# somepago/DCR

Hardware: NVIDIA H100
Metric: embed+top-k query images/sec (higher is better)
Workload: dtype bf16

## Files before the change

dcr_b200/csrc/conv3x3_halo.cu:

```cuda
#include <cuda_bf16.h>

#include <algorithm>
#include <cstring>

#include "dcr_internal.cuh"
#include "host_util.cuh"
#include "ptx.cuh"

namespace dcr {

namespace {

constexpr int kHM = 128;
constexpr int kHK = 64;
constexpr int kSlabBytes = kHM * 128;
constexpr int kHThreads = 288;

struct HaloMaps {
  CUtensorMap a;
  CUtensorMap w;
  CUtensorMap out;
};

struct HaloParams {
  int H, W, Wp, R, N, cblocks;
  int tiles_per_img, num_tiles;
  int a_bufs, w_stages;
  uint32_t halo_bytes;
  uint32_t a_buf_bytes;
  const float* scale;
  const float* bias;
// ... 2 lines not shown

DCR_DEVICE void tma_store_commit_() { asm volatile("cp.async.bulk.commit_group;" ::: "memory"); }
DCR_DEVICE void tma_store_wait_read_() { asm volatile("cp.async.bulk.wait_group.read 0;" ::: "memory"); }
DCR_DEVICE void tma_store_wait_all_() { asm volatile("cp.async.bulk.wait_group 0;" ::: "memory"); }
DCR_DEVICE uint32_t pack_bf16_(float a, float b) {
  __nv_bfloat162 p = __floats2bfloat162_rn(a, b);
  return *reinterpret_cast<uint32_t*>(&p);
}

template <int BN, bool kRW>
__global__ void __launch_bounds__(kHThreads, 1)
    conv3x3_halo_kernel(const __grid_constant__ HaloMaps maps, const HaloParams p) {
  extern __shared__ __align__(1024) uint8_t smem_raw[];
  uint8_t* smem = reinterpret_cast<uint8_t*>((reinterpret_cast<uintptr_t>(smem_raw) + 1023) & ~uintptr_t(1023));
  constexpr int kWStage = BN * 128;
  constexpr int kChunksPerWarp = BN / 64;
  uint8_t* a_ring = smem;
  uint8_t* w_ring = a_ring + p.a_bufs * p.a_buf_bytes;
  uint8_t* out_stage = w_ring + (kRW ? 9 * p.cblocks : p.w_stages) * kWStage;
  uint8_t* acc_xpose = out_stage + (BN / 64) * kSlabBytes;
  float* sb = reinterpret_cast<float*>(acc_xpose + 8 * kAccXposeWarpBytes);
  uint64_t* bars = reinterpret_cast<uint64_t*>(sb + 2 * BN);
  uint64_t* a_full = bars;
  uint64_t* a_empty = bars + 4;
  uint64_t* w_full = bars + 8;
  uint64_t* w_empty = bars + 16;

  const uint32_t warp = threadIdx.x >> 5, lane = threadIdx.x & 31;
  if (warp == 8 && lane == 0) {
    tma_prefetch_desc(&maps.a);
    tma_prefetch_desc(&maps.w);
    tma_prefetch_desc(&maps.out);
  }
  if (warp == 0 && lane == 0) {
    for (int s = 0; s < p.a_bufs; ++s) {
      mbar_init(&a_full[s], 1);
      mbar_init(&a_empty[s], 8);
    }
    for (int s = 0; s < (kRW ? 1 : p.w_stages); ++s) {
      mbar_init(&w_full[s], 1);
      mbar_init(&w_empty[s], 8);
    }
    fence_mbar_init();
  }
  __syncthreads();

  if (warp == 8) {
    {
      PipeState as(p.a_bufs), ws(kRW ? 1 : p.w_stages);
      if constexpr (kRW) {
        if (elect_one()) {
          mbar_arrive_expect_tx(&w_full[0], 9 * p.cblocks * kWStage);
          for (int t = 0; t < 9 * p.cblocks; ++t)
            tma_load_2d(w_ring + t * kWStage, &maps.w, &w_full[0], t * kHK, 0, kEvictLast);
        }
        __syncwarp();
      }
      for (int tile = blockIdx.x; tile < p.num_tiles; tile += gridDim.x) {
        const int b = tile / p.tiles_per_img;
        const int p0 = (tile - b * p.tiles_per_img) * p.R;
        for (int cb = 0; cb < p.cblocks; ++cb, as.next()) {
          const uint32_t sa = as.s, pha = as.ph;
          mbar_wait(&a_empty[sa], pha ^ 1);
// ... 4 lines not shown
          __syncwarp();
          if constexpr (kRW) continue;
          for (int tap = 0; tap < 9; ++tap, ws.next()) {
            const uint32_t sw = ws.s, phw = ws.ph;
            mbar_wait(&w_empty[sw], phw ^ 1);
            if (elect_one()) {
              mbar_arrive_expect_tx(&w_full[sw], kWStage);
              tma_load_2d(w_ring + sw * kWStage, &maps.w, &w_full[sw], (tap * p.cblocks + cb) * kHK, 0, kEvictLast);
            }
            __syncwarp();
          }
        }
      }
    }
  } else {
    const uint32_t ewarp = warp;
    const uint32_t quad = warp & 3;
    const uint32_t half = ewarp >> 2;
    const uint32_t m = quad * 32 + lane;
    const uint32_t etid = ewarp * 32 + lane;
    const uint32_t xacc = smem_u32(acc_xpose) + warp * kAccXposeWarpBytes;
    const uint32_t a_base = smem_u32(a_ring);
    const uint32_t w_base = smem_u32(w_ring) + half * (BN / 2) * 128;
    const uint32_t row_bytes = static_cast<uint32_t>(p.Wp) * 128u;
    PipeState as(p.a_bufs), ws(kRW ? 1 : p.w_stages);
    if constexpr (kRW) mbar_wait(&w_full[0], 0);
    const int pl = static_cast<int>(m) / p.Wp, ql = static_cast<int>(m) - pl * p.Wp;
    const bool valid = ql < p.W && pl < p.R;
    const uint32_t srow = static_cast<uint32_t>(pl * p.W + ql);
    const uint32_t sb_addr = smem_u32(sb), stage_addr = smem_u32(out_stage);
    for (int c = etid; c < BN; c += 256) {
      st_shared_f32(sb_addr + c * 4, (p.scale && c < p.N) ? p.scale[c] : 1.f);
      st_shared_f32(sb_addr + (BN + c) * 4, (p.bias && c < p.N) ? p.bias[c] : 0.f);
    }
    for (int tile = blockIdx.x; tile < p.num_tiles; tile += gridDim.x) {
      const int b = tile / p.tiles_per_img;
      const int p0 = (tile - b * p.tiles_per_img) * p.R;
      if (etid == 0) tma_store_wait_read_();
      asm volatile("bar.sync 1, 256;" ::: "memory");
      WgAcc<BN / 2> acc;
      uint32_t accumulate = 0;
      for (int cb = 0; cb < p.cblocks; ++cb, as.next()) {
        const uint32_t sa = as.s;
        mbar_wait(&a_full[sa], as.ph);
        const uint32_t a_buf = a_base + sa * p.a_buf_bytes;
#pragma unroll 1
        for (int tap = 0; tap < 9; ++tap) {
          const int r = tap / 3, s = tap - 3 * r;
          uint32_t sw = 0;
          if constexpr (!kRW) {
            sw = ws.s;
            mbar_wait(&w_full[sw], ws.ph);
          } else {
            sw = static_cast<uint32_t>(tap * p.cblocks + cb);
          }
          const uint32_t a_addr = a_buf + r * row_bytes + s * 128u;
          const uint32_t b_addr = w_base + sw * kWStage;
          wgmma_fence();
#pragma unroll
          for (int k = 0; k < kHK / 16; ++k) acc.mma(a_addr + 32 * k, wgmma_desc_sw128(b_addr + 32 * k), accumulate | k);
          wgmma_commit();
          wgmma_wait<0>();
          accumulate = 1;
          if constexpr (!kRW) {
            if (lane == 0) mbar_arrive(&w_empty[sw]);
            ws.next();
          }
        }
        if (lane == 0) mbar_arrive(&a_empty[sa]);
      }
      acc.fence_regs();
#pragma unroll
      for (int ci = 0; ci < kChunksPerWarp; ++ci) {
        const int ch = half * kChunksPerWarp + ci;
        uint32_t r[32];
        acc.rows32(ci, r, xacc, lane);
        if (ch * 32 >= p.N) continue;
        float y[32];
#pragma unroll
        for (int c = 0; c < 32; c += 4) {
          const float4 sc = ld_shared_f4(sb_addr + (ch * 32 + c) * 4);
          const float4 bi = ld_shared_f4(sb_addr + (BN + ch * 32 + c) * 4);
          y[c + 0] = fmaf(__uint_as_float(r[c + 0]), sc.x, bi.x);
          y[c + 1] = fmaf(__uint_as_float(r[c + 1]), sc.y, bi.y);
          y[c + 2] = fmaf(__uint_as_float(r[c + 2]), sc.z, bi.z);
          y[c + 3] = fmaf(__uint_as_float(r[c + 3]), sc.w, bi.w);
        }
        if (p.act == 1) {
#pragma unroll
          for (int c = 0; c < 32; ++c) y[c] = fmaxf(y[c], 0.f);
        }
        const uint32_t dst = stage_addr + (ch >> 1) * kSlabBytes + srow * 128;
        const uint32_t sw = srow & 7;
#pragma unroll
        for (int j = 0; j < 4; ++j) {
          uint4 v;
          v.x = pack_bf16_(y[j * 8 + 0], y[j * 8 + 1]);
          v.y = pack_bf16_(y[j * 8 + 2], y[j * 8 + 3]);
          v.z = pack_bf16_(y[j * 8 + 4], y[j * 8 + 5]);
          v.w = pack_bf16_(y[j * 8 + 6], y[j * 8 + 7]);
          if (valid) st_shared_v4(dst + ((((ch & 1) * 4 + j) ^ sw) << 4), v);
        }
        __syncwarp();
      }
      fence_proxy_async();
      asm volatile("bar.sync 2, 256;" ::: "memory");
      if (etid == 0) {
        for (int sl = 0; sl < BN / 64; ++sl)
          if (sl * 64 < p.N) tma_store_4d(&maps.out, out_stage + sl * kSlabBytes, p.out_col_off + sl * 64, 0, p0, b);
        tma_store_commit_();
      }
    }
    if (etid == 0) tma_store_wait_all_();
  }

}

template <int BN, bool kRW>
int launch_halo(const HaloMaps& maps, HaloParams& p, int num_sms, size_t max_smem, cudaStream_t stream) {
  constexpr size_t kWStage = static_cast<size_t>(BN) * 128;
  const size_t fixed = 1024 + static_cast<size_t>(BN / 64) * kSlabBytes + 8 * kAccXposeWarpBytes + 2 * BN * 4 + 256;
  const size_t abuf = p.a_buf_bytes;
  size_t smem = 0;
  if constexpr (kRW) {
    const size_t wres = static_cast<size_t>(9) * p.cblocks * kWStage;
    DCR_REQUIRE(max_smem >= fixed + wres + 2 * abuf, "conv3x3_halo: resident weights do not fit");
    p.a_bufs = static_cast<int>(std::min<size_t>(4, (max_smem - fixed - wres) / abuf));
    p.w_stages = 0;
    smem = fixed + wres + static_cast<size_t>(p.a_bufs) * abuf;
  } else {
    p.a_bufs = 2;
    DCR_REQUIRE(max_smem >= fixed + 2 * abuf + 3 * kWStage, "conv3x3_halo: not enough shared memory");
    p.w_stages = static_cast<int>(std::min<size_t>(8, (max_smem - fixed - 2 * abuf) / kWStage));
    if (max_smem >= fixed + 3 * abuf + 6 * kWStage) {
      p.a_bufs = 3;
      p.w_stages = static_cast<int>(std::min<size_t>(8, (max_smem - fixed - 3 * abuf) / kWStage));
// ... 59 lines not shown
```

dcr_b200/csrc/conv_gemm.cu:

```cuda
#include <cuda_bf16.h>

#include <algorithm>
#include <cstring>

#include "dcr_internal.cuh"
#include "host_util.cuh"
#include "ptx.cuh"

namespace dcr {

namespace {

constexpr int kBM = 128;
constexpr int kBK = 64;
constexpr int kThreads = 288;
constexpr int kAccXposeBytes = 8 * kAccXposeWarpBytes;
constexpr int kAStage = kBM * kBK * 2;
constexpr int kXposePitch = 80;
constexpr int kXposeWarpBytes = 32 * kXposePitch;
constexpr int kXposeBytes = 8 * kXposeWarpBytes;

struct GemmMaps {
  CUtensorMap a[3];
  CUtensorMap w[3];
  CUtensorMap out;
  CUtensorMap res;
};

struct GemmParams {
  int M, N;
// ... 2 lines not shown
  int term_a[kMaxGemmTerms], term_w[kMaxGemmTerms];
  int P, Q, stride, pad_h, pad_w;
  int num_m_tiles, num_n_tiles, stages;
  const float* scale;
  const float* bias;
  const __nv_bfloat16* res;
  int ld_res, res_planes;
  long long res_plane_stride;
  __nv_bfloat16* out;
  int ld_out, out_col_off, out_planes;
  long long out_plane_stride;
  float* out_f32;
  int ld_out_f32;
  int act;
  int tma_epi;
  int n_out_bufs;
  int n_res_bufs;
  int fast_gelu;
  int n_fastest;
  int a_resident;
};

DCR_DEVICE float gelu_erf_fast(float y) {
  const float ax = fabsf(y) * 0.70710678118654752440f;
  float t;
  asm("rcp.approx.ftz.f32 %0, %1;" : "=f"(t) : "f"(fmaf(0.3275911f, ax, 1.f)));
  float e;
  asm("ex2.approx.ftz.f32 %0, %1;" : "=f"(e) : "f"(-1.4426950408889634f * ax * ax));
  float poly = fmaf(1.061405429f, t, -1.453152027f);
  poly = fmaf(poly, t, 1.421413741f);
  poly = fmaf(poly, t, -0.284496736f);
  poly = fmaf(poly, t, 0.254829592f);
// ... 29 lines not shown
               : "memory");
}
DCR_DEVICE void tma_store_commit() { asm volatile("cp.async.bulk.commit_group;" ::: "memory"); }
DCR_DEVICE void tma_store_wait_read() { asm volatile("cp.async.bulk.wait_group.read 0;" ::: "memory"); }
DCR_DEVICE void tma_store_wait_all() { asm volatile("cp.async.bulk.wait_group 0;" ::: "memory"); }

template <int BN, bool kIm2col, int kEpi>
__global__ void __launch_bounds__(kThreads, 1)
    gemm_bf16_kernel(const __grid_constant__ GemmMaps maps, const GemmParams p) {
  extern __shared__ __align__(1024) uint8_t smem_raw[];
  uint8_t* smem = reinterpret_cast<uint8_t*>((reinterpret_cast<uintptr_t>(smem_raw) + 1023) & ~uintptr_t(1023));
  constexpr bool kTma = kEpi != 0;
  constexpr int kBStage = BN * kBK * 2;
  constexpr int kStageBytes = kAStage + kBStage;
  constexpr int kStagingBytes = (BN / 64) * kBM * 128;
  constexpr int kChunksPerWarp = BN / 64;
  const int stages = p.stages;
  const int k_iters = p.n_terms * p.taps * p.cblocks;
  const bool a_res = p.a_resident != 0;
  const int stage_bytes = a_res ? kBStage : kStageBytes;
  const int num_n_tiles = p.num_n_tiles;
  uint8_t* smem_ares = smem;
  uint8_t* smem_ab = smem + (a_res ? k_iters * kAStage : 0);
  uint8_t* out_stage = smem_ab + stages * stage_bytes;
  uint8_t* res_stage = out_stage + (kTma ? p.n_out_bufs * kStagingBytes : kXposeBytes);
  uint8_t* acc_xpose = res_stage + p.n_res_bufs * kStagingBytes;
  float* sb = reinterpret_cast<float*>(acc_xpose + kAccXposeBytes);
  uint64_t* bars = reinterpret_cast<uint64_t*>(sb + (a_res ? 2 * num_n_tiles * BN : 4 * BN));
  uint64_t* full = bars;
  uint64_t* empty = bars + 12;
  uint64_t* res_full = bars + 28;
  uint64_t* a_full = bars + 10;
  uint64_t* a_empty = bars + 11;

  const uint32_t warp = threadIdx.x >> 5, lane = threadIdx.x & 31;
  const int M = p.M, N = p.N, num_m_tiles = p.num_m_tiles;
  const bool has_res = p.res != nullptr;
  const int num_tiles = num_m_tiles * p.num_n_tiles;
  const int unit = static_cast<int>(blockIdx.x), n_units = static_cast<int>(gridDim.x);
  const int t_first = a_res ? static_cast<int>(static_cast<long long>(num_tiles) * blockIdx.x / gridDim.x) : unit;
  const int t_end = a_res ? static_cast<int>(static_cast<long long>(num_tiles) * (blockIdx.x + 1) / gridDim.x) : num_tiles;
  const int t_step = a_res ? 1 : n_units;
  const bool n_fast = p.n_fastest != 0;
  auto tile_m = [&](int t) {
    return a_res ? t / num_n_tiles : (n_fast ? t / num_n_tiles : t % num_m_tiles);
  };
  auto tile_n = [&](int t) { return (a_res || n_fast) ? t % num_n_tiles : t / num_m_tiles; };

  if (warp == 8 && lane == 0) {
    tma_prefetch_desc(&maps.out);
    tma_prefetch_desc(&maps.res);
    for (int i = 0; i < 3; ++i) {
      tma_prefetch_desc(&maps.a[i]);
      tma_prefetch_desc(&maps.w[i]);
    }
  }
  if (warp == 0 && lane == 0) {
    for (int s = 0; s < stages; ++s) {
      mbar_init(&full[s], 1);
      mbar_init(&empty[s], 8);
    }
    for (int b = 0; b < 2; ++b) mbar_init(&res_full[b], 1);
    mbar_init(a_full, 1);
    mbar_init(a_empty, 8);
    fence_mbar_init();
  }
  __syncthreads();

  if (warp == 8) {
    {
      const int n_terms = p.n_terms, taps = p.taps, kw = p.kw, cblocks = p.cblocks;
      PipeState st(stages);
      int res_m = -1;
      uint32_t a_seg = 0;
      for (int tile = t_first; tile < t_end; tile += t_step) {
        const int m0 = tile_m(tile) * kBM;
        const int n0 = tile_n(tile) * BN;
        if (a_res) {
          if (m0 != res_m) {
            res_m = m0;
            mbar_wait(a_empty, (a_seg & 1) ^ 1);
            if (elect_one()) {
              mbar_arrive_expect_tx(a_full, k_iters * kAStage);
              for (int ki = 0; ki < k_iters; ++ki)
                tma_load_2d(smem_ares + ki * kAStage, &maps.a[p.term_a[0]], a_full, ki * kBK, m0, kEvictFirst);
            }
            __syncwarp();
            ++a_seg;
          }
          for (int ki = 0; ki < k_iters; ++ki, st.next()) {
            const uint32_t s = st.s;
            mbar_wait(&empty[s], st.ph ^ 1);
            if (elect_one()) {
              mbar_arrive_expect_tx(&full[s], kBStage);
              tma_load_2d(smem_ab + s * kBStage, &maps.w[p.term_w[0]], &full[s], ki * kBK, n0, kEvictLast);
            }
            __syncwarp();
          }
          continue;
        }
// ... 19 lines not shown
                uint8_t* sa = smem_ab + s * kStageBytes;
                if constexpr (kIm2col) {
                  tma_load_im2col_4d(sa, ma, &full[s], cb * kBK, w0, h0, img, static_cast<uint16_t>(sx),
                                          static_cast<uint16_t>(r));
                } else
                  tma_load_2d(sa, ma, &full[s], cb * kBK, m0, kEvictNormal);
                tma_load_2d(sa + kAStage, mw, &full[s], (tap * cblocks + cb) * kBK, n0, kEvictNormal);
              }
              __syncwarp();
            }
          }
        }
      }
    }
  } else {
    const uint32_t ewarp = warp;
    const uint32_t quad = warp & 3;
    const uint32_t half = ewarp >> 2;
    const uint32_t row = quad * 32 + lane;
    const uint32_t etid = ewarp * 32 + lane;
    const uint32_t xacc = smem_u32(acc_xpose) + warp * kAccXposeWarpBytes;
    const int act = p.act;
    uint32_t tc = 0;
    PipeState st(stages);
    const uint32_t a_base = smem_u32(a_res ? smem_ares : smem_ab);
    const uint32_t b_base = smem_u32(a_res ? smem_ab : smem_ab + kAStage) + half * (BN / 2) * 128;
    int res_m_c = -1;
    uint32_t a_seg = 0;
    auto load_residual = [&](int tile_idx, uint32_t rbuf) {
      const int rm0 = tile_m(tile_idx) * kBM;
      const int rn0 = tile_n(tile_idx) * BN;
      int slabs = 0;
      for (int sl = 0; sl < BN / 64; ++sl)
        if (rn0 + sl * 64 < N) ++slabs;
      mbar_arrive_expect_tx(&res_full[rbuf], slabs * kBM * 128);
      for (int sl = 0; sl < BN / 64; ++sl)
        if (rn0 + sl * 64 < N)
          tma_load_2d(res_stage + rbuf * kStagingBytes + sl * kBM * 128, &maps.res, &res_full[rbuf], rn0 + sl * 64, rm0,
                         kEvictFirst);
    };
    if (kTma && has_res && etid == 0 && t_first < t_end) load_residual(t_first, 0);
    const bool two_out = p.n_out_bufs == 2;
    const uint32_t sb_addr = smem_u32(sb), out_addr = smem_u32(out_stage), res_addr = smem_u32(res_stage);
    int staged_n0 = -1;
    uint32_t sbsel = 1;
    if (a_res) {
      const int npad = num_n_tiles * BN;
      for (int c = etid; c < npad; c += 256) {
        st_shared_f32(sb_addr + c * 4, (p.scale && c < N) ? p.scale[c] : 1.f);
        st_shared_f32(sb_addr + (npad + c) * 4, (p.bias && c < N) ? p.bias[c] : 0.f);
      }
      asm volatile("bar.sync 1, 256;" ::: "memory");
    }
    for (int tile = t_first; tile < t_end; tile += t_step, ++tc) {
      const int m0 = tile_m(tile) * kBM;
      const int n0 = tile_n(tile) * BN;
      uint8_t* ostage = out_stage + (two_out ? (tc & 1) : 0) * kStagingBytes;
      const uint32_t ostage_addr = out_addr + (two_out ? (tc & 1) : 0) * kStagingBytes;
      const uint32_t rstage_addr = res_addr + (tc & 1) * kStagingBytes;
      if constexpr (kTma) {
        if (etid == 0) {
          if (!two_out) tma_store_wait_read();
          if (has_res && tile + t_step < t_end) load_residual(tile + t_step, (tc & 1) ^ 1);
        }
      }
      const bool restage = !a_res && n0 != staged_n0;
      if (restage) {
        sbsel ^= 1;
        staged_n0 = n0;
        for (int c = etid; c < BN; c += 256) {
          const int n = n0 + c;
          st_shared_f32(sb_addr + (sbsel * 2 * BN + c) * 4, (p.scale && n < N) ? p.scale[n] : 1.f);
          st_shared_f32(sb_addr + (sbsel * 2 * BN + BN + c) * 4, (p.bias && n < N) ? p.bias[n] : 0.f);
        }
      }
      if (restage || (kTma && !two_out)) asm volatile("bar.sync 1, 256;" ::: "memory");
      const uint32_t s_scale = a_res ? sb_addr + n0 * 4 : sb_addr + sbsel * 2 * BN * 4;
      const uint32_t s_bias = s_scale + (a_res ? num_n_tiles * BN : BN) * 4;
      bool last_of_m = false;
      if (a_res) {
        const int mt = tile_m(tile);
        if (mt != res_m_c) {
          res_m_c = mt;
          mbar_wait(a_full, a_seg & 1);
          ++a_seg;
        }
        last_of_m = (tile + t_step >= t_end) || tile_m(tile + t_step) != mt;
      }
      WgAcc<BN / 2> acc;
      uint32_t prev_s = 0;
      for (int ki = 0; ki < k_iters; ++ki, st.next()) {
        const uint32_t s = st.s;
        mbar_wait(&full[s], st.ph);
        const uint32_t a_addr = a_base + (a_res ? static_cast<uint32_t>(ki) * kAStage : s * kStageBytes);
        const uint32_t b_addr = b_base + s * static_cast<uint32_t>(stage_bytes);
        wgmma_fence();
#pragma unroll
        for (int k = 0; k < kBK / 16; ++k) acc.mma(a_addr + 32 * k, wgmma_desc_sw128(b_addr + 32 * k), (ki | k) != 0);
        wgmma_commit();
        wgmma_wait<1>();
        if (ki > 0 && lane == 0) mbar_arrive(&empty[prev_s]);
        prev_s = s;
      }
      wgmma_wait<0>();
      acc.fence_regs();
      if (lane == 0) {
        mbar_arrive(&empty[prev_s]);
        if (last_of_m) mbar_arrive(a_empty);
      }
      if (kTma && has_res) mbar_wait(&res_full[tc & 1], (tc >> 1) & 1);
      const int m = m0 + static_cast<int>(row);
      const bool row_ok = m < M;
#pragma unroll
      for (int ci = 0; ci < kChunksPerWarp; ++ci) {
        const int ch = half * kChunksPerWarp + ci;
        uint32_t r[32];
        acc.rows32(ci, r, xacc, lane);
        const int nc = n0 + ch * 32;
        if (nc >= N) continue;
        float y[32];
#pragma unroll
        for (int c = 0; c < 32; c += 4) {
          const float4 sc = ld_shared_f4(s_scale + (ch * 32 + c) * 4);
          const float4 bi = ld_shared_f4(s_bias + (ch * 32 + c) * 4);
          y[c + 0] = fmaf(__uint_as_float(r[c + 0]), sc.x, bi.x);
          y[c + 1] = fmaf(__uint_as_float(r[c + 1]), sc.y, bi.y);
          y[c + 2] = fmaf(__uint_as_float(r[c + 2]), sc.z, bi.z);
          y[c + 3] = fmaf(__uint_as_float(r[c + 3]), sc.w, bi.w);
        }
        if constexpr (kTma) {
          const uint32_t srow = ostage_addr + (ch >> 1) * kBM * 128 + row * 128;
          const uint32_t rrow = rstage_addr + (ch >> 1) * kBM * 128 + row * 128;
          const uint32_t sw = row & 7;
          if (has_res) {
#pragma unroll
            for (int j = 0; j < 4; ++j) {
              const uint4 rv = ld_shared_v4(rrow + ((((ch & 1) * 4 + j) ^ sw) << 4));
              const uint32_t w[4] = {rv.x, rv.y, rv.z, rv.w};
#pragma unroll
              for (int e = 0; e < 4; ++e) {
                y[j * 8 + 2 * e] += __uint_as_float(w[e] << 16);
                y[j * 8 + 2 * e + 1] += __uint_as_float(w[e] & 0xffff0000u);
              }
            }
          }
#pragma unroll
          for (int c = 0; c < 32; ++c) y[c] = (kEpi == 3) ? gelu_tanh_fast(y[c]) : apply_act(y[c], kEpi - 1);
#pragma unroll
          for (int j = 0; j < 4; ++j) {
            uint4 v;
            v.x = pack_bf16(y[j * 8 + 0], y[j * 8 + 1]);
            v.y = pack_bf16(y[j * 8 + 2], y[j * 8 + 3]);
// ... 72 lines not shown
                const int piece = t * 32 + static_cast<int>(lane), r = piece >> 2, part = piece & 3;
                if (m_w0 + r < M && part * 8 < nvalid)
                  *reinterpret_cast<uint4*>(obase + static_cast<size_t>(m_w0 + r) * p.ld_out + part * 8) =
                      ld_shared_v4(xw + r * kXposePitch + part * 16);
              }
              if (pl + 1 < p.out_planes) {
#pragma unroll
                for (int c = 0; c < 32; ++c) y[c] -= __bfloat162float(__float2bfloat16_rn(y[c]));
              }
            }
          }
        }
      }
      if constexpr (kTma) {
        fence_proxy_async();
        if (two_out && etid == 0) tma_store_wait_read();
        asm volatile("bar.sync 2, 256;" ::: "memory");
        if (etid == 0) {
          for (int sl = 0; sl < BN / 64; ++sl)
            if (n0 + sl * 64 < N && m0 < M) tma_store_2d(&maps.out, ostage + sl * kBM * 128, p.out_col_off + n0 + sl * 64, m0);
          tma_store_commit();
        }
      }
    }
  }

  if (kTma && warp == 0 && lane == 0) tma_store_wait_all();
}

bool wants_a_resident(const GemmParams& p, int BN, bool im2col, size_t max_smem) {
  const int k_iters_h = p.n_terms * p.taps * p.cblocks;
  if (!(!im2col && p.tma_epi && p.n_terms == 1 && p.num_n_tiles >= 2 && (p.res != nullptr || p.num_n_tiles >= 4) &&
        k_iters_h * kAStage <= 64 * 1024 && p.num_n_tiles * BN <= 4096))
    return false;
  const size_t staging = static_cast<size_t>(BN / 64) * kBM * 128;
  const size_t need = 1024 + static_cast<size_t>(2) * p.num_n_tiles * BN * 4 + static_cast<size_t>(k_iters_h) * kAStage + 256 +
                      static_cast<size_t>(1 + (p.res ? 2 : 0)) * staging + kAccXposeBytes + 3 * static_cast<size_t>(BN) * kBK * 2;
  return need <= max_smem;
}

template <int BN, bool kIm2col, int kEpi>
int launch(const GemmMaps& maps, GemmParams& p, int num_sms, size_t max_smem, cudaStream_t stream) {
  constexpr int kStageBytes = kAStage + BN * kBK * 2;
  constexpr size_t kStagingBytes = static_cast<size_t>(BN / 64) * kBM * 128;
  p.n_res_bufs = (p.tma_epi && p.res) ? 2 : 0;
  p.n_out_bufs = p.tma_epi ? 2 : 0;
  const int k_iters_h = p.n_terms * p.taps * p.cblocks;
  p.a_resident = (kEpi != 0 && wants_a_resident(p, BN, kIm2col, max_smem)) ? 1 : 0;
  const size_t sb_bytes = p.a_resident ? static_cast<size_t>(2) * p.num_n_tiles * BN * 4 : static_cast<size_t>(4) * BN * 4;
  const size_t ares_bytes = p.a_resident ? static_cast<size_t>(k_iters_h) * kAStage : 0;
  auto fixed_for = [&](int nout, int nres) {
    return 1024 + sb_bytes + ares_bytes + 256 + static_cast<size_t>(nout + nres) * kStagingBytes + (p.tma_epi ? 0 : kXposeBytes) +
           kAccXposeBytes;
  };
  const size_t stage_bytes = p.a_resident ? static_cast<size_t>(BN) * kBK * 2 : static_cast<size_t>(kStageBytes);
  if (p.tma_epi && (fixed_for(p.n_out_bufs, p.n_res_bufs) + 3 * stage_bytes > max_smem)) p.n_out_bufs = 1;
  const size_t fixed = fixed_for(p.n_out_bufs, p.n_res_bufs);
  DCR_REQUIRE(max_smem > fixed + 2 * stage_bytes, "gemm: not enough shared memory");
  int stages = static_cast<int>((max_smem - fixed) / stage_bytes);
  stages = std::min(stages, 8);
  p.stages = stages;
  const size_t smem = fixed + static_cast<size_t>(stages) * stage_bytes;
  auto kern = gemm_bf16_kernel<BN, kIm2col, kEpi>;
  static bool attr_set_dev[64] = {};
  int cur_dev = 0;
  DCR_CUDA_CHECK(cudaGetDevice(&cur_dev));
  bool& attr_set = attr_set_dev[cur_dev & 63];
  if (!attr_set) {
    DCR_CUDA_CHECK(cudaFuncSetAttribute(kern, cudaFuncAttributeMaxDynamicSharedMemorySize, static_cast<int>(max_smem)));
    attr_set = true;
  }
  {
    const int tiles = p.num_m_tiles * p.num_n_tiles;
// ... 23 lines not shown
  const int P = (d.H + 2 * d.pad_h - d.kh) / d.stride + 1;
  const int Q = (d.W + 2 * d.pad_w - d.kw) / d.stride + 1;
  const long long M = static_cast<long long>(d.B) * P * Q;
  DCR_REQUIRE(M > 0 && M < (1ll << 31), "conv_gemm: M out of range");
  const int cblocks = (d.C + kBK - 1) / kBK;
  const int ktot = d.kh * d.kw * cblocks * kBK;

  GemmMaps maps;
  memset(&maps, 0, sizeof(maps));
  int a_planes = 0, w_planes = 0;
  for (int t = 0; t < d.n_terms; ++t) {
    a_planes = std::max(a_planes, d.term_a[t] + 1);
    w_planes = std::max(w_planes, d.term_w[t] + 1);
  }
  DCR_REQUIRE(a_planes <= 3 && w_planes <= 3, "conv_gemm: at most 3 planes");
  int BN = d.N <= 64 ? 64 : (d.N <= 128 ? 128 : 256);
  const bool single_plane = d.out && d.out_planes <= 1 && !d.out_f32 && (!d.res || d.res_planes <= 1);
  if (BN == 256 && single_plane && (d.res != nullptr || static_cast<long long>(d.kh) * d.kw * d.C <= 256)) BN = 128;
  {
    const long long m_tiles = (M + kBM - 1) / kBM;
    while (BN > 64 && ktot >= 1024 && m_tiles * ((d.N + BN - 1) / BN) * 4 <= di->num_sms) BN /= 2;
  }
  for (int pl = 0; pl < 3; ++pl) {
    const int pa = std::min(pl, a_planes - 1), pw = std::min(pl, w_planes - 1);
    const __nv_bfloat16* abase = d.in + pa * d.in_plane_stride;
    if (im2col) {
      DCR_REQUIRE(windowed || d.ld_in == d.C, "conv_gemm: im2col input must be dense NHWC (ld_in == C)");
      if (int rc = make_tmap_im2col_bf16(&maps.a[pl], abase, d.B, d.H, d.W, d.C, d.pad_h, d.pad_w, d.kh, d.kw, d.stride,
                                         kBK, kBM, d.in_stride_w, d.in_stride_h, d.in_stride_n))
        return rc;
    } else {
      if (int rc = make_tmap_2d_bf16(&maps.a[pl], abase, M, d.C, d.ld_in, kBM, kBK)) return rc;
    }
// ... 52 lines not shown
  } else {
    maps.out = maps.w[0];
    maps.res = maps.w[0];
  }
  DCR_REQUIRE(p.out == nullptr || (p.ld_out % 8 == 0 && p.out_col_off % 8 == 0), "conv_gemm: output leading dim / offset must be multiples of 8");
  DCR_REQUIRE(p.res == nullptr || p.ld_res % 8 == 0, "conv_gemm: residual leading dim must be a multiple of 8");
  DCR_REQUIRE(p.out_f32 == nullptr || p.ld_out_f32 % 4 == 0, "conv_gemm: fp32 output leading dim must be a multiple of 4");

  const int epi = p.tma_epi ? 1 + p.act : 0;

#define DCR_LAUNCH_E(BNv, E)                                                                      \
  (im2col ? launch<BNv, true, E>(maps, p, di->num_sms, di->max_smem_optin, stream)              \
          : launch<BNv, false, E>(maps, p, di->num_sms, di->max_smem_optin, stream))
#define DCR_LAUNCH(BNv)                                                                          \
  (epi == 0 ? DCR_LAUNCH_E(BNv, 0)                                                                \
            : (epi == 1 ? DCR_LAUNCH_E(BNv, 1) : (epi == 2 ? DCR_LAUNCH_E(BNv, 2) : (epi == 3 ? DCR_LAUNCH_E(BNv, 3) : DCR_LAUNCH_E(BNv, 4)))))
  switch (BN) {
    case 64: return DCR_LAUNCH(64);
    case 128: return DCR_LAUNCH(128);
    case 256: return DCR_LAUNCH(256);
    default: return set_error(-1, "conv_gemm: unsupported BN %d", BN);
  }
#undef DCR_LAUNCH_E
#undef DCR_LAUNCH
}

}
```

dcr_b200/csrc/ptx.cuh:

```cuda
#pragma once
#include <cstdint>
#include <cuda.h>
#include <cuda_runtime.h>

namespace dcr {

#define DCR_DEVICE __device__ __forceinline__

DCR_DEVICE uint32_t smem_u32(const void* p) { return static_cast<uint32_t>(__cvta_generic_to_shared(p)); }

DCR_DEVICE bool elect_one() {
  uint32_t pred = 0;
  asm volatile(
      "{\n\t.reg .pred P;\n\t"
      "elect.sync _|P, 0xffffffff;\n\t"
      "selp.u32 %0, 1, 0, P;\n\t}\n"
      : "=r"(pred));
  return pred != 0;
}

DCR_DEVICE void mbar_init(uint64_t* bar, uint32_t count) {
  asm volatile("mbarrier.init.shared::cta.b64 [%0], %1;" ::"r"(smem_u32(bar)), "r"(count) : "memory");
}
DCR_DEVICE void fence_mbar_init() { asm volatile("fence.mbarrier_init.release.cluster;" ::: "memory"); }
DCR_DEVICE void fence_proxy_async() { asm volatile("fence.proxy.async.shared::cta;" ::: "memory"); }

DCR_DEVICE void mbar_arrive(uint64_t* bar) {
  asm volatile("mbarrier.arrive.shared::cta.b64 _, [%0];" ::"r"(smem_u32(bar)) : "memory");
}
DCR_DEVICE void mbar_arrive_expect_tx(uint64_t* bar, uint32_t bytes) {
  asm volatile("mbarrier.arrive.expect_tx.shared::cta.b64 _, [%0], %1;" ::"r"(smem_u32(bar)), "r"(bytes) : "memory");
}
DCR_DEVICE bool mbar_try_wait(uint64_t* bar, uint32_t parity) {
  uint32_t ok;
  asm volatile(
      "{\n\t.reg .pred P;\n\t"
      "mbarrier.try_wait.parity.shared::cta.b64 P, [%1], %2;\n\t"
      "selp.u32 %0, 1, 0, P;\n\t}\n"
      : "=r"(ok)
      : "r"(smem_u32(bar)), "r"(parity)
      : "memory");
  return ok != 0;
}
// ... 5 lines not shown
      "@P bra DONE_%=;\n\t"
      "bra WAIT_%=;\n\t"
      "DONE_%=:\n\t}\n" ::"r"(smem_u32(bar)),
      "r"(parity)
      : "memory");
}
struct PipeState {
  uint32_t s, ph, n;
  DCR_DEVICE explicit PipeState(uint32_t stages) : s(0), ph(0), n(stages) {}
  DCR_DEVICE void next() {
    if (++s == n) {
      s = 0;
      ph ^= 1;
    }
  }
};

DCR_DEVICE void tma_prefetch_desc(const void* tmap) {
  asm volatile("prefetch.tensormap [%0];" ::"l"(reinterpret_cast<uint64_t>(tmap)) : "memory");
}

constexpr uint64_t kEvictNormal = 0x1000000000000000ull;
constexpr uint64_t kEvictFirst = 0x12F0000000000000ull;
constexpr uint64_t kEvictLast = 0x14F0000000000000ull;

DCR_DEVICE void tma_load_2d(void* dst, const void* tmap, uint64_t* bar, int c0, int c1, uint64_t hint) {
  asm volatile(
      "cp.async.bulk.tensor.2d.shared::cluster.global.mbarrier::complete_tx::bytes.L2::cache_hint"
      " [%0], [%1, {%3, %4}], [%2], %5;" ::"r"(smem_u32(dst)),
      "l"(reinterpret_cast<uint64_t>(tmap)), "r"(smem_u32(bar)), "r"(c0), "r"(c1), "l"(hint)
      : "memory");
// ... 150 lines not shown
```

Baseline: 2945.

## Ping-pong two consumer warpgroups over alternating tiles with register rebalancing

Both the conv GEMM and halo conv3x3 kernels move from two warpgroups splitting one tile's N dimension to two consumer warpgroups that each own full-width tiles and alternate between tiles. A turn mbarrier orders their MMA phases so one group's epilogue overlaps the other's mainloop. A producer warpgroup is added with setmaxnreg to shift registers to the consumers. Each group gets its own output staging buffer, and the residual tile now loads into that buffer. BN=256 is dropped and wgmma waits keep one or two groups in flight. The aim is to hide epilogue time and keep tensor cores busy, at the cost of more register pressure per consumer and more complex barrier phase bookkeeping.

```diff
diff --git a/dcr_b200/csrc/conv3x3_halo.cu b/dcr_b200/csrc/conv3x3_halo.cu
--- a/dcr_b200/csrc/conv3x3_halo.cu
+++ b/dcr_b200/csrc/conv3x3_halo.cu
@@ -14,7 +14,8 @@
 constexpr int kHM = 128;
 constexpr int kHK = 64;
 constexpr int kSlabBytes = kHM * 128;
-constexpr int kHThreads = 288;
+constexpr int kHThreads = 384;
+constexpr int kHConsumerRegs = 224, kHProducerRegs = 56;
 
 struct HaloMaps {
   CUtensorMap a;
@@ -47,17 +48,17 @@
   extern __shared__ __align__(1024) uint8_t smem_raw[];
   uint8_t* smem = reinterpret_cast<uint8_t*>((reinterpret_cast<uintptr_t>(smem_raw) + 1023) & ~uintptr_t(1023));
   constexpr int kWStage = BN * 128;
-  constexpr int kChunksPerWarp = BN / 64;
+  constexpr int kStageBytes = (BN / 64) * kSlabBytes;
   uint8_t* a_ring = smem;
   uint8_t* w_ring = a_ring + p.a_bufs * p.a_buf_bytes;
   uint8_t* out_stage = w_ring + (kRW ? 9 * p.cblocks : p.w_stages) * kWStage;
-  uint8_t* acc_xpose = out_stage + (BN / 64) * kSlabBytes;
-  float* sb = reinterpret_cast<float*>(acc_xpose + 8 * kAccXposeWarpBytes);
+  float* sb = reinterpret_cast<float*>(out_stage + 2 * kStageBytes);
   uint64_t* bars = reinterpret_cast<uint64_t*>(sb + 2 * BN);
   uint64_t* a_full = bars;
   uint64_t* a_empty = bars + 4;
   uint64_t* w_full = bars + 8;
   uint64_t* w_empty = bars + 16;
+  uint64_t* turn = bars + 24;
 
   const uint32_t warp = threadIdx.x >> 5, lane = threadIdx.x & 31;
   if (warp == 8 && lane == 0) {
@@ -68,18 +69,20 @@
   if (warp == 0 && lane == 0) {
     for (int s = 0; s < p.a_bufs; ++s) {
       mbar_init(&a_full[s], 1);
-      mbar_init(&a_empty[s], 8);
+      mbar_init(&a_empty[s], 4);
     }
     for (int s = 0; s < (kRW ? 1 : p.w_stages); ++s) {
       mbar_init(&w_full[s], 1);
-      mbar_init(&w_empty[s], 8);
-    }
+      mbar_init(&w_empty[s], 4);
+    }
+    for (int g = 0; g < 2; ++g) mbar_init(&turn[g], 4);
     fence_mbar_init();
   }
   __syncthreads();
 
-  if (warp == 8) {
-    {
+  if (warp >= 8) {
+    wg_regs_dec<kHProducerRegs>();
+    if (warp == 8) {
       PipeState as(p.a_bufs), ws(kRW ? 1 : p.w_stages);
       if constexpr (kRW) {
         if (elect_one()) {
@@ -114,32 +117,47 @@
       }
     }
   } else {
-    const uint32_t ewarp = warp;
+    wg_regs_inc<kHConsumerRegs>();
     const uint32_t quad = warp & 3;
-    const uint32_t half = ewarp >> 2;
-    const uint32_t m = quad * 32 + lane;
-    const uint32_t etid = ewarp * 32 + lane;
-    const uint32_t xacc = smem_u32(acc_xpose) + warp * kAccXposeWarpBytes;
+    const uint32_t wg = warp >> 2;
+    const uint32_t gtid = (warp & 3) * 32 + lane;
     const uint32_t a_base = smem_u32(a_ring);
-    const uint32_t w_base = smem_u32(w_ring) + half * (BN / 2) * 128;
+    const uint32_t w_base = smem_u32(w_ring);
     const uint32_t row_bytes = static_cast<uint32_t>(p.Wp) * 128u;
+    const int k_groups = 9 * p.cblocks;
     PipeState as(p.a_bufs), ws(kRW ? 1 : p.w_stages);
     if constexpr (kRW) mbar_wait(&w_full[0], 0);
-    const int pl = static_cast<int>(m) / p.Wp, ql = static_cast<int>(m) - pl * p.Wp;
-    const bool valid = ql < p.W && pl < p.R;
-    const uint32_t srow = static_cast<uint32_t>(pl * p.W + ql);
-    const uint32_t sb_addr = smem_u32(sb), stage_addr = smem_u32(out_stage);
-    for (int c = etid; c < BN; c += 256) {
-      st_shared_f32(sb_addr + c * 4, (p.scale && c < p.N) ? p.scale[c] : 1.f);
-      st_shared_f32(sb_addr + (BN + c) * 4, (p.bias && c < p.N) ? p.bias[c] : 0.f);
-    }
-    for (int tile = blockIdx.x; tile < p.num_tiles; tile += gridDim.x) {
+    const uint32_t r0 = lane >> 2, c0 = 2 * (lane & 3);
+    uint32_t srow[4];
+    bool valid[4];
+#pragma unroll
+    for (int g = 0; g < 4; ++g) {
+      const int m = static_cast<int>(quad * 32 + r0 + 8 * g);
+      const int pl = m / p.Wp, ql = m - pl * p.Wp;
+      valid[g] = ql < p.W && pl < p.R;
+      srow[g] = static_cast<uint32_t>(pl * p.W + ql);
+    }
+    const uint32_t sb_addr = smem_u32(sb), stage_addr = smem_u32(out_stage) + wg * kStageBytes;
+    uint8_t* ostage = out_stage + wg * kStageBytes;
+    for (int c = warp * 32 + lane; c < BN; c += 256) {
+      st_shared_f32(sb_addr + c * 4, p.scale ? p.scale[c] : 1.f);
+      st_shared_f32(sb_addr + (BN + c) * 4, p.bias ? p.bias[c] : 0.f);
+    }
+    named_bar_sync(5, 256);
+    if (wg == 1) {
+      as.skip(p.cblocks);
+      if constexpr (!kRW) ws.skip(k_groups);
+    }
+    uint32_t tc = 0;
+    for (int tile = blockIdx.x + wg * gridDim.x; tile < p.num_tiles; tile += 2 * gridDim.x, ++tc) {
       const int b = tile / p.tiles_per_img;
       const int p0 = (tile - b * p.tiles_per_img) * p.R;
-      if (etid == 0) tma_store_wait_read_();
-      asm volatile("bar.sync 1, 256;" ::: "memory");
-      WgAcc<BN / 2> acc;
-      uint32_t accumulate = 0;
+      if (gtid == 0) tma_store_wait_read_();
+      named_bar_sync(1 + 2 * wg, 128);
+      if (wg == 1 || tc > 0) mbar_wait(&turn[wg], (wg == 1 ? tc : tc - 1) & 1);
+      WgAcc<BN> acc;
+      uint32_t prev_w = 0, prev_a = 0;
+      bool prev_a_last = false;
       for (int cb = 0; cb < p.cblocks; ++cb, as.next()) {
         const uint32_t sa = as.s;
         mbar_wait(&a_full[sa], as.ph);
@@ -158,68 +176,58 @@
           const uint32_t b_addr = w_base + sw * kWStage;
           wgmma_fence();
 #pragma unroll
-          for (int k = 0; k < kHK / 16; ++k) acc.mma(a_addr + 32 * k, wgmma_desc_sw128(b_addr + 32 * k), accumulate | k);
+          for (int k = 0; k < kHK / 16; ++k) acc.mma(a_addr + 32 * k, wgmma_desc_sw128(b_addr + 32 * k), (cb | tap | k) != 0);
           wgmma_commit();
-          wgmma_wait<0>();
-          accumulate = 1;
-          if constexpr (!kRW) {
-            if (lane == 0) mbar_arrive(&w_empty[sw]);
-            ws.next();
+          const bool last = cb == p.cblocks - 1 && tap == 8;
+          if (last && lane == 0) mbar_arrive(&turn[wg ^ 1]);
+          wgmma_wait<1>();
+          if ((cb | tap) != 0 && lane == 0) {
+            if constexpr (!kRW) mbar_arrive(&w_empty[prev_w]);
+            if (prev_a_last) mbar_arrive(&a_empty[prev_a]);
           }
+          prev_w = sw;
+          prev_a = sa;
+          prev_a_last = tap == 8;
+          if constexpr (!kRW) ws.next();
         }
-        if (lane == 0) mbar_arrive(&a_empty[sa]);
-      }
+      }
+      wgmma_wait<0>();
       acc.fence_regs();
-#pragma unroll
-      for (int ci = 0; ci < kChunksPerWarp; ++ci) {
-        const int ch = half * kChunksPerWarp + ci;
-        uint32_t r[32];
-        acc.rows32(ci, r, xacc, lane);
-        if (ch * 32 >= p.N) continue;
-        float y[32];
-#pragma unroll
-        for (int c = 0; c < 32; c += 4) {
-          const float4 sc = ld_shared_f4(sb_addr + (ch * 32 + c) * 4);
-          const float4 bi = ld_shared_f4(sb_addr + (BN + ch * 32 + c) * 4);
-          y[c + 0] = fmaf(__uint_as_float(r[c + 0]), sc.x, bi.x);
-          y[c + 1] = fmaf(__uint_as_float(r[c + 1]), sc.y, bi.y);
-          y[c + 2] = fmaf(__uint_as_float(r[c + 2]), sc.z, bi.z);
-          y[c + 3] = fmaf(__uint_as_float(r[c + 3]), sc.w, bi.w);
+      if (lane == 0) {
+        if constexpr (!kRW) mbar_arrive(&w_empty[prev_w]);
+        mbar_arrive(&a_empty[prev_a]);
+      }
+      as.skip(p.cblocks);
+      if constexpr (!kRW) ws.skip(k_groups);
+      acc.for_each_pair(lane, [&](uint32_t row, uint32_t col, float v0, float v1) {
+        const uint32_t g = (row - r0) >> 3;
+        const float2 sc = ld_shared_f2(sb_addr + col * 4);
+        const float2 bi = ld_shared_f2(sb_addr + (BN + col) * 4);
+        float y0 = fmaf(v0, sc.x, bi.x), y1 = fmaf(v1, sc.y, bi.y);
+        if (p.act == 1) {
+          y0 = fmaxf(y0, 0.f);
+          y1 = fmaxf(y1, 0.f);
         }
-        if (p.act == 1) {
-#pragma unroll
-          for (int c = 0; c < 32; ++c) y[c] = fmaxf(y[c], 0.f);
-        }
-        const uint32_t dst = stage_addr + (ch >> 1) * kSlabBytes + srow * 128;
-        const uint32_t sw = srow & 7;
-#pragma unroll
-        for (int j = 0; j < 4; ++j) {
-          uint4 v;
-          v.x = pack_bf16_(y[j * 8 + 0], y[j * 8 + 1]);
-          v.y = pack_bf16_(y[j * 8 + 2], y[j * 8 + 3]);
-          v.z = pack_bf16_(y[j * 8 + 4], y[j * 8 + 5]);
-          v.w = pack_bf16_(y[j * 8 + 6], y[j * 8 + 7]);
-          if (valid) st_shared_v4(dst + ((((ch & 1) * 4 + j) ^ sw) << 4), v);
-        }
-        __syncwarp();
-      }
+        const uint32_t chunk = (col & 63) >> 3;
+        if (valid[g])
+          st_shared_u32(stage_addr + (col >> 6) * kSlabBytes + srow[g] * 128 + ((chunk ^ (srow[g] & 7)) << 4) + c0 * 2,
+                        pack_bf16_(y0, y1));
+      });
       fence_proxy_async();
-      asm volatile("bar.sync 2, 256;" ::: "memory");
-      if (etid == 0) {
-        for (int sl = 0; sl < BN / 64; ++sl)
-          if (sl * 64 < p.N) tma_store_4d(&maps.out, out_stage + sl * kSlabBytes, p.out_col_off + sl * 64, 0, p0, b);
+      named_bar_sync(2 + 2 * wg, 128);
+      if (gtid == 0) {
+        for (int sl = 0; sl < BN / 64; ++sl) tma_store_4d(&maps.out, ostage + sl * kSlabBytes, p.out_col_off + sl * 64, 0, p0, b);
         tma_store_commit_();
       }
     }
-    if (etid == 0) tma_store_wait_all_();
-  }
-
+    if (gtid == 0) tma_store_wait_all_();
+  }
 }
 
 template <int BN, bool kRW>
 int launch_halo(const HaloMaps& maps, HaloParams& p, int num_sms, size_t max_smem, cudaStream_t stream) {
   constexpr size_t kWStage = static_cast<size_t>(BN) * 128;
-  const size_t fixed = 1024 + static_cast<size_t>(BN / 64) * kSlabBytes + 8 * kAccXposeWarpBytes + 2 * BN * 4 + 256;
+  const size_t fixed = 1024 + static_cast<size_t>(2) * (BN / 64) * kSlabBytes + 2 * BN * 4 + 256;
   const size_t abuf = p.a_buf_bytes;
   size_t smem = 0;
   if constexpr (kRW) {
diff --git a/dcr_b200/csrc/conv_gemm.cu b/dcr_b200/csrc/conv_gemm.cu
--- a/dcr_b200/csrc/conv_gemm.cu
+++ b/dcr_b200/csrc/conv_gemm.cu
@@ -13,7 +13,9 @@
 
 constexpr int kBM = 128;
 constexpr int kBK = 64;
-constexpr int kThreads = 288;
+constexpr int kThreads = 384;
+constexpr int consumer_regs(int epi) { return epi == 0 ? 240 : 224; }
+constexpr int producer_regs(int epi) { return epi == 0 ? 24 : 56; }
 constexpr int kAccXposeBytes = 8 * kAccXposeWarpBytes;
 constexpr int kAStage = kBM * kBK * 2;
 constexpr int kXposePitch = 80;
@@ -46,8 +48,6 @@
   int ld_out_f32;
   int act;
   int tma_epi;
-  int n_out_bufs;
-  int n_res_bufs;
   int fast_gelu;
   int n_fastest;
   int a_resident;
@@ -107,7 +107,8 @@
   constexpr int kBStage = BN * kBK * 2;
   constexpr int kStageBytes = kAStage + kBStage;
   constexpr int kStagingBytes = (BN / 64) * kBM * 128;
-  constexpr int kChunksPerWarp = BN / 64;
+  constexpr int kChunksPerWarp = BN / 32;
+  constexpr int kPend = BN <= 64 ? 2 : 1;
   const int stages = p.stages;
   const int k_iters = p.n_terms * p.taps * p.cblocks;
   const bool a_res = p.a_resident != 0;
@@ -116,14 +117,14 @@
   uint8_t* smem_ares = smem;
   uint8_t* smem_ab = smem + (a_res ? k_iters * kAStage : 0);
   uint8_t* out_stage = smem_ab + stages * stage_bytes;
-  uint8_t* res_stage = out_stage + (kTma ? p.n_out_bufs * kStagingBytes : kXposeBytes);
-  uint8_t* acc_xpose = res_stage + p.n_res_bufs * kStagingBytes;
+  uint8_t* acc_xpose = out_stage + (kTma ? 2 * kStagingBytes : kXposeBytes);
   float* sb = reinterpret_cast<float*>(acc_xpose + kAccXposeBytes);
-  uint64_t* bars = reinterpret_cast<uint64_t*>(sb + (a_res ? 2 * num_n_tiles * BN : 4 * BN));
+  uint64_t* bars = reinterpret_cast<uint64_t*>(sb + (a_res ? 2 * num_n_tiles * BN : 8 * BN));
   uint64_t* full = bars;
   uint64_t* empty = bars + 12;
   uint64_t* res_full = bars + 28;
-  uint64_t* a_full = bars + 10;
+  uint64_t* turn = bars + 30;
+  uint64_t* a_full = bars + 9;
   uint64_t* a_empty = bars + 11;
 
   const uint32_t warp = threadIdx.x >> 5, lane = threadIdx.x & 31;
@@ -151,17 +152,22 @@
   if (warp == 0 && lane == 0) {
     for (int s = 0; s < stages; ++s) {
       mbar_init(&full[s], 1);
-      mbar_init(&empty[s], 8);
-    }
-    for (int b = 0; b < 2; ++b) mbar_init(&res_full[b], 1);
-    mbar_init(a_full, 1);
+      mbar_init(&empty[s], 4);
+    }
+    for (int b = 0; b < 2; ++b) {
+      mbar_init(&res_full[b], 1);
+      mbar_init(&turn[b], 4);
+    }
+    mbar_init(&a_full[0], 1);
+    mbar_init(&a_full[1], 1);
     mbar_init(a_empty, 8);
     fence_mbar_init();
   }
   __syncthreads();
 
-  if (warp == 8) {
-    {
+  if (warp >= 8) {
+    wg_regs_dec<producer_regs(kEpi)>();
+    if (warp == 8) {
       const int n_terms = p.n_terms, taps = p.taps, kw = p.kw, cblocks = p.cblocks;
       PipeState st(stages);
       int res_m = -1;
@@ -174,9 +180,9 @@
             res_m = m0;
             mbar_wait(a_empty, (a_seg & 1) ^ 1);
             if (elect_one()) {
-              mbar_arrive_expect_tx(a_full, k_iters * kAStage);
+              mbar_arrive_expect_tx(&a_full[a_seg & 1], k_iters * kAStage);
               for (int ki = 0; ki < k_iters; ++ki)
-                tma_load_2d(smem_ares + ki * kAStage, &maps.a[p.term_a[0]], a_full, ki * kBK, m0, kEvictFirst);
+                tma_load_2d(smem_ares + ki * kAStage, &maps.a[p.term_a[0]], &a_full[a_seg & 1], ki * kBK, m0, kEvictFirst);
             }
             __syncwarp();
             ++a_seg;
@@ -226,34 +232,33 @@
       }
     }
   } else {
+    wg_regs_inc<consumer_regs(kEpi)>();
     const uint32_t ewarp = warp;
     const uint32_t quad = warp & 3;
-    const uint32_t half = ewarp >> 2;
+    const uint32_t wg = ewarp >> 2;
     const uint32_t row = quad * 32 + lane;
     const uint32_t etid = ewarp * 32 + lane;
+    const uint32_t gtid = etid & 127;
+    const uint32_t bar_top = 1 + 2 * wg, bar_end = bar_top + 1;
     const uint32_t xacc = smem_u32(acc_xpose) + warp * kAccXposeWarpBytes;
     const int act = p.act;
     uint32_t tc = 0;
     PipeState st(stages);
     const uint32_t a_base = smem_u32(a_res ? smem_ares : smem_ab);
-    const uint32_t b_base = smem_u32(a_res ? smem_ab : smem_ab + kAStage) + half * (BN / 2) * 128;
+    const uint32_t b_base = smem_u32(a_res ? smem_ab : smem_ab + kAStage);
     int res_m_c = -1;
-    uint32_t a_seg = 0;
-    auto load_residual = [&](int tile_idx, uint32_t rbuf) {
+    const int m_first = t_first < t_end ? tile_m(t_first) : 0;
+    auto load_residual = [&](int tile_idx, uint8_t* dst, uint64_t* bar) {
       const int rm0 = tile_m(tile_idx) * kBM;
       const int rn0 = tile_n(tile_idx) * BN;
       int slabs = 0;
       for (int sl = 0; sl < BN / 64; ++sl)
         if (rn0 + sl * 64 < N) ++slabs;
-      mbar_arrive_expect_tx(&res_full[rbuf], slabs * kBM * 128);
+      mbar_arrive_expect_tx(bar, slabs * kBM * 128);
       for (int sl = 0; sl < BN / 64; ++sl)
-        if (rn0 + sl * 64 < N)
-          tma_load_2d(res_stage + rbuf * kStagingBytes + sl * kBM * 128, &maps.res, &res_full[rbuf], rn0 + sl * 64, rm0,
-                         kEvictFirst);
+        if (rn0 + sl * 64 < N) tma_load_2d(dst + sl * kBM * 128, &maps.res, bar, rn0 + sl * 64, rm0, kEvictFirst);
     };
-    if (kTma && has_res && etid == 0 && t_first < t_end) load_residual(t_first, 0);
-    const bool two_out = p.n_out_bufs == 2;
-    const uint32_t sb_addr = smem_u32(sb), out_addr = smem_u32(out_stage), res_addr = smem_u32(res_stage);
+    const uint32_t sb_addr = smem_u32(sb) + (a_res ? 0 : wg * 4 * BN * 4);
     int staged_n0 = -1;
     uint32_t sbsel = 1;
     if (a_res) {
@@ -262,45 +267,49 @@
         st_shared_f32(sb_addr + c * 4, (p.scale && c < N) ? p.scale[c] : 1.f);
         st_shared_f32(sb_addr + (npad + c) * 4, (p.bias && c < N) ? p.bias[c] : 0.f);
       }
-      asm volatile("bar.sync 1, 256;" ::: "memory");
-    }
-    for (int tile = t_first; tile < t_end; tile += t_step, ++tc) {
+      named_bar_sync(5, 256);
+    }
+    if (wg == 1) st.skip(k_iters);
+    for (int tile = t_first + static_cast<int>(wg) * t_step; tile < t_end; tile += 2 * t_step, ++tc) {
       const int m0 = tile_m(tile) * kBM;
       const int n0 = tile_n(tile) * BN;
-      uint8_t* ostage = out_stage + (two_out ? (tc & 1) : 0) * kStagingBytes;
-      const uint32_t ostage_addr = out_addr + (two_out ? (tc & 1) : 0) * kStagingBytes;
-      const uint32_t rstage_addr = res_addr + (tc & 1) * kStagingBytes;
-      if constexpr (kTma) {
-        if (etid == 0) {
-          if (!two_out) tma_store_wait_read();
-          if (has_res && tile + t_step < t_end) load_residual(tile + t_step, (tc & 1) ^ 1);
-        }
+      uint8_t* ostage = out_stage + wg * kStagingBytes;
+      const uint32_t ostage_addr = smem_u32(ostage);
+      if (kTma && gtid == 0) {
+        tma_store_wait_read();
+        if (has_res) load_residual(tile, ostage, &res_full[wg]);
       }
       const bool restage = !a_res && n0 != staged_n0;
       if (restage) {
         sbsel ^= 1;
         staged_n0 = n0;
-        for (int c = etid; c < BN; c += 256) {
+        for (int c = gtid; c < BN; c += 128) {
           const int n = n0 + c;
           st_shared_f32(sb_addr + (sbsel * 2 * BN + c) * 4, (p.scale && n < N) ? p.scale[n] : 1.f);
           st_shared_f32(sb_addr + (sbsel * 2 * BN + BN + c) * 4, (p.bias && n < N) ? p.bias[n] : 0.f);
         }
       }
-      if (restage || (kTma && !two_out)) asm volatile("bar.sync 1, 256;" ::: "memory");
+      if (restage || kTma) named_bar_sync(bar_top, 128);
       const uint32_t s_scale = a_res ? sb_addr + n0 * 4 : sb_addr + sbsel * 2 * BN * 4;
       const uint32_t s_bias = s_scale + (a_res ? num_n_tiles * BN : BN) * 4;
-      bool last_of_m = false;
+      bool a_release = false;
+      uint32_t a_release_cnt = 1;
       if (a_res) {
         const int mt = tile_m(tile);
         if (mt != res_m_c) {
           res_m_c = mt;
-          mbar_wait(a_full, a_seg & 1);
-          ++a_seg;
-        }
-        last_of_m = (tile + t_step >= t_end) || tile_m(tile + t_step) != mt;
-      }
-      WgAcc<BN / 2> acc;
-      uint32_t prev_s = 0;
+          const int seg = mt - m_first;
+          mbar_wait(&a_full[seg & 1], (seg >> 1) & 1);
+        }
+        const int next = tile + 2 * t_step;
+        a_release = next >= t_end || tile_m(next) != mt;
+        const bool alone = (tile - t_step < t_first || tile_m(tile - t_step) != mt) &&
+                           (tile + t_step >= t_end || tile_m(tile + t_step) != mt);
+        a_release_cnt = alone ? 2 : 1;
+      }
+      if (wg == 1 || tc > 0) mbar_wait(&turn[wg], (wg == 1 ? tc : tc - 1) & 1);
+      WgAcc<BN> acc;
+      uint32_t pend[kPend] = {};
       for (int ki = 0; ki < k_iters; ++ki, st.next()) {
         const uint32_t s = st.s;
         mbar_wait(&full[s], st.ph);
@@ -310,22 +319,28 @@
 #pragma unroll
         for (int k = 0; k < kBK / 16; ++k) acc.mma(a_addr + 32 * k, wgmma_desc_sw128(b_addr + 32 * k), (ki | k) != 0);
         wgmma_commit();
-        wgmma_wait<1>();
-        if (ki > 0 && lane == 0) mbar_arrive(&empty[prev_s]);
-        prev_s = s;
+        if (ki == k_iters - 1 && lane == 0) mbar_arrive(&turn[wg ^ 1]);
+        wgmma_wait<kPend>();
+        if (ki >= kPend && lane == 0) mbar_arrive(&empty[pend[0]]);
+#pragma unroll
+        for (int j = 0; j + 1 < kPend; ++j) pend[j] = pend[j + 1];
+        pend[kPend - 1] = s;
       }
       wgmma_wait<0>();
       acc.fence_regs();
       if (lane == 0) {
-        mbar_arrive(&empty[prev_s]);
-        if (last_of_m) mbar_arrive(a_empty);
-      }
-      if (kTma && has_res) mbar_wait(&res_full[tc & 1], (tc >> 1) & 1);
+#pragma unroll
+        for (int j = 0; j < kPend; ++j)
+          if (k_iters - kPend + j >= 0) mbar_arrive(&empty[pend[j]]);
+        if (a_release) mbar_arrive_cnt(a_empty, a_release_cnt);
+      }
+      st.skip(k_iters);
+      if (kTma && has_res) mbar_wait(&res_full[wg], tc & 1);
       const int m = m0 + static_cast<int>(row);
       const bool row_ok = m < M;
 #pragma unroll
       for (int ci = 0; ci < kChunksPerWarp; ++ci) {
-        const int ch = half * kChunksPerWarp + ci;
+        const int ch = ci;
         uint32_t r[32];
         acc.rows32(ci, r, xacc, lane);
         const int nc = n0 + ch * 32;
@@ -342,12 +357,11 @@
         }
         if constexpr (kTma) {
           const uint32_t srow = ostage_addr + (ch >> 1) * kBM * 128 + row * 128;
-          const uint32_t rrow = rstage_addr + (ch >> 1) * kBM * 128 + row * 128;
           const uint32_t sw = row & 7;
           if (has_res) {
 #pragma unroll
             for (int j = 0; j < 4; ++j) {
-              const uint4 rv = ld_shared_v4(rrow + ((((ch & 1) * 4 + j) ^ sw) << 4));
+              const uint4 rv = ld_shared_v4(srow + ((((ch & 1) * 4 + j) ^ sw) << 4));
               const uint32_t w[4] = {rv.x, rv.y, rv.z, rv.w};
 #pragma unroll
               for (int e = 0; e < 4; ++e) {
@@ -450,9 +464,8 @@
       }
       if constexpr (kTma) {
         fence_proxy_async();
-        if (two_out && etid == 0) tma_store_wait_read();
-        asm volatile("bar.sync 2, 256;" ::: "memory");
-        if (etid == 0) {
+        named_bar_sync(bar_end, 128);
+        if (gtid == 0) {
           for (int sl = 0; sl < BN / 64; ++sl)
             if (n0 + sl * 64 < N && m0 < M) tma_store_2d(&maps.out, ostage + sl * kBM * 128, p.out_col_off + n0 + sl * 64, m0);
           tma_store_commit();
@@ -461,7 +474,7 @@
     }
   }
 
-  if (kTma && warp == 0 && lane == 0) tma_store_wait_all();
+  if (kTma && (warp == 0 || warp == 4) && lane == 0) tma_store_wait_all();
 }
 
 bool wants_a_resident(const GemmParams& p, int BN, bool im2col, size_t max_smem) {
@@ -471,7 +484,7 @@
     return false;
   const size_t staging = static_cast<size_t>(BN / 64) * kBM * 128;
   const size_t need = 1024 + static_cast<size_t>(2) * p.num_n_tiles * BN * 4 + static_cast<size_t>(k_iters_h) * kAStage + 256 +
-                      static_cast<size_t>(1 + (p.res ? 2 : 0)) * staging + kAccXposeBytes + 3 * static_cast<size_t>(BN) * kBK * 2;
+                      2 * staging + kAccXposeBytes + 3 * static_cast<size_t>(BN) * kBK * 2;
   return need <= max_smem;
 }
 
@@ -479,20 +492,13 @@
 int launch(const GemmMaps& maps, GemmParams& p, int num_sms, size_t max_smem, cudaStream_t stream) {
   constexpr int kStageBytes = kAStage + BN * kBK * 2;
   constexpr size_t kStagingBytes = static_cast<size_t>(BN / 64) * kBM * 128;
-  p.n_res_bufs = (p.tma_epi && p.res) ? 2 : 0;
-  p.n_out_bufs = p.tma_epi ? 2 : 0;
   const int k_iters_h = p.n_terms * p.taps * p.cblocks;
   p.a_resident = (kEpi != 0 && wants_a_resident(p, BN, kIm2col, max_smem)) ? 1 : 0;
-  const size_t sb_bytes = p.a_resident ? static_cast<size_t>(2) * p.num_n_tiles * BN * 4 : static_cast<size_t>(4) * BN * 4;
+  const size_t sb_bytes = p.a_resident ? static_cast<size_t>(2) * p.num_n_tiles * BN * 4 : static_cast<size_t>(8) * BN * 4;
   const size_t ares_bytes = p.a_resident ? static_cast<size_t>(k_iters_h) * kAStage : 0;
-  auto fixed_for = [&](int nout, int nres) {
-    return 1024 + sb_bytes + ares_bytes + 256 + static_cast<size_t>(nout + nres) * kStagingBytes + (p.tma_epi ? 0 : kXposeBytes) +
-           kAccXposeBytes;
-  };
+  const size_t fixed = 1024 + sb_bytes + ares_bytes + 256 + (p.tma_epi ? 2 * kStagingBytes : kXposeBytes) + kAccXposeBytes;
   const size_t stage_bytes = p.a_resident ? static_cast<size_t>(BN) * kBK * 2 : static_cast<size_t>(kStageBytes);
-  if (p.tma_epi && (fixed_for(p.n_out_bufs, p.n_res_bufs) + 3 * stage_bytes > max_smem)) p.n_out_bufs = 1;
-  const size_t fixed = fixed_for(p.n_out_bufs, p.n_res_bufs);
-  DCR_REQUIRE(max_smem > fixed + 2 * stage_bytes, "gemm: not enough shared memory");
+  DCR_REQUIRE(max_smem > fixed + 3 * stage_bytes, "gemm: not enough shared memory");
   int stages = static_cast<int>((max_smem - fixed) / stage_bytes);
   stages = std::min(stages, 8);
   p.stages = stages;
@@ -546,9 +552,8 @@
     w_planes = std::max(w_planes, d.term_w[t] + 1);
   }
   DCR_REQUIRE(a_planes <= 3 && w_planes <= 3, "conv_gemm: at most 3 planes");
-  int BN = d.N <= 64 ? 64 : (d.N <= 128 ? 128 : 256);
-  const bool single_plane = d.out && d.out_planes <= 1 && !d.out_f32 && (!d.res || d.res_planes <= 1);
-  if (BN == 256 && single_plane && (d.res != nullptr || static_cast<long long>(d.kh) * d.kw * d.C <= 256)) BN = 128;
+  int BN = d.N <= 64 ? 64 : 128;
+  if (d.act == 3) BN = 64;
   {
     const long long m_tiles = (M + kBM - 1) / kBM;
     while (BN > 64 && ktot >= 1024 && m_tiles * ((d.N + BN - 1) / BN) * 4 <= di->num_sms) BN /= 2;
@@ -631,11 +636,10 @@
           : launch<BNv, false, E>(maps, p, di->num_sms, di->max_smem_optin, stream))
 #define DCR_LAUNCH(BNv)                                                                          \
   (epi == 0 ? DCR_LAUNCH_E(BNv, 0)                                                                \
-            : (epi == 1 ? DCR_LAUNCH_E(BNv, 1) : (epi == 2 ? DCR_LAUNCH_E(BNv, 2) : (epi == 3 ? DCR_LAUNCH_E(BNv, 3) : DCR_LAUNCH_E(BNv, 4)))))
+            : (epi == 1 ? DCR_LAUNCH_E(BNv, 1) : (epi == 2 ? DCR_LAUNCH_E(BNv, 2) : (epi == 3 ? DCR_LAUNCH_E(BNv, 3) : DCR_LAUNCH_E(64, 4)))))
   switch (BN) {
     case 64: return DCR_LAUNCH(64);
     case 128: return DCR_LAUNCH(128);
-    case 256: return DCR_LAUNCH(256);
     default: return set_error(-1, "conv_gemm: unsupported BN %d", BN);
   }
 #undef DCR_LAUNCH_E
diff --git a/dcr_b200/csrc/ptx.cuh b/dcr_b200/csrc/ptx.cuh
--- a/dcr_b200/csrc/ptx.cuh
+++ b/dcr_b200/csrc/ptx.cuh
@@ -27,6 +27,9 @@
 
 DCR_DEVICE void mbar_arrive(uint64_t* bar) {
   asm volatile("mbarrier.arrive.shared::cta.b64 _, [%0];" ::"r"(smem_u32(bar)) : "memory");
+}
+DCR_DEVICE void mbar_arrive_cnt(uint64_t* bar, uint32_t count) {
+  asm volatile("mbarrier.arrive.shared::cta.b64 _, [%0], %1;" ::"r"(smem_u32(bar)), "r"(count) : "memory");
 }
 DCR_DEVICE void mbar_arrive_expect_tx(uint64_t* bar, uint32_t bytes) {
   asm volatile("mbarrier.arrive.expect_tx.shared::cta.b64 _, [%0], %1;" ::"r"(smem_u32(bar)), "r"(bytes) : "memory");
@@ -62,7 +65,19 @@
       ph ^= 1;
     }
   }
+  DCR_DEVICE void skip(int k) {
+    for (int i = 0; i < k; ++i) next();
+  }
 };
+
+template <int kRegs>
+DCR_DEVICE void wg_regs_dec() { asm volatile("setmaxnreg.dec.sync.aligned.u32 %0;" ::"n"(kRegs)); }
+template <int kRegs>
+DCR_DEVICE void wg_regs_inc() { asm volatile("setmaxnreg.inc.sync.aligned.u32 %0;" ::"n"(kRegs)); }
+
+DCR_DEVICE void named_bar_sync(uint32_t id, uint32_t threads) {
+  asm volatile("bar.sync %0, %1;" ::"r"(id), "r"(threads) : "memory");
+}
 
 DCR_DEVICE void tma_prefetch_desc(const void* tmap) {
   asm volatile("prefetch.tensormap [%0];" ::"l"(reinterpret_cast<uint64_t>(tmap)) : "memory");
```

Result: faster. 3471, median of 6 (+17.9%).
